# OmerKerner/noLZSS

Hardware: AMD Instinct MI355X
Metric: bases/sec factorized (1 GB sigma=4 DNA) + HBM GB/s fraction (higher is better)
Workload: dtype u32; 1 GPU; dna1g: one 2^30-base synthetic DNA sequence per GPU (sigma=4, 40% copied blocks, 1% substitutions), full factorization to (start,length,ref) records in HBM; bases_per_gpu=1073741824, parallelism=1 independent sequence shard(s), all-gather of counts

## Files before the change

include/nolzss_hip.h:

```cpp
#ifndef NOLZSS_HIP_H
#define NOLZSS_HIP_H

#include <stddef.h>
#include <stdint.h>

#ifdef __cplusplus
extern "C" {
#endif

typedef struct nolzss_factor {
    uint64_t start;
    uint64_t length;
    uint64_t ref;
} nolzss_factor;

#define NOLZSS_RC_MASK (1ULL << 63)

enum {
    NOLZSS_OK = 0,
    NOLZSS_ERR_INVALID_ARGUMENT = 1,
    NOLZSS_ERR_RUNTIME = 2,
    NOLZSS_ERR_NOMEM = 3,
    NOLZSS_ERR_DEVICE = 4,
    NOLZSS_ERR_IO = 5,
// ... 257 lines not shown
    uint64_t z, n_literals;
    uint64_t total_length;
    const uint64_t *target_lengths;
    int32_t device;
    uint64_t device_bytes;
} nolzss_rlz_archive_summary;
int nolzss_rlz_archive_open_records(const uint8_t *block, size_t block_len, const nolzss_factor *records, size_t z,
                                    const uint8_t *literals, size_t n_literals, const uint64_t *target_lengths,
                                    size_t k, int device, nolzss_rlz_archive **h);
int nolzss_rlz_archive_info(const nolzss_rlz_archive *h, nolzss_rlz_archive_summary *info);
int nolzss_rlz_archive_extract(const nolzss_rlz_archive *h, const nolzss_rlz_range *ranges, size_t q, uint8_t **bytes,
                               uint64_t **offsets, uint64_t *total);
int nolzss_rlz_archive_extract_device(const nolzss_rlz_archive *h, const nolzss_rlz_range *ranges, size_t q,
                                      void *d_out, size_t d_out_capacity, void *stream, uint64_t *total);
int nolzss_rlz_archive_close(nolzss_rlz_archive *h);

typedef struct nolzss_rlz_index nolzss_rlz_index;
typedef struct nolzss_rlz_index_summary {
    uint64_t num_references, block_length, index_length;
    int32_t with_rc, device;
    uint32_t prefix_syms;
    uint64_t device_bytes;
} nolzss_rlz_index_summary;
int nolzss_rlz_index_open(const char *const *refs, const size_t *ref_lens, size_t m, int with_rc,
                          uint32_t prefix_syms, int device, nolzss_rlz_index **h);
int nolzss_rlz_index_open_fasta(const char *reference_fasta_path, int with_rc, int sanitize_mode,
                                uint32_t prefix_syms, int device, nolzss_rlz_index **h);
int nolzss_rlz_index_info(const nolzss_rlz_index *h, nolzss_rlz_index_summary *info);
int nolzss_rlz_index_factorize(const nolzss_rlz_index *h, const char *const *targets, const size_t *target_lens,
                               size_t k, int want_factors, nolzss_rlz_result *out);
int nolzss_rlz_index_codes(const nolzss_rlz_index *h, const char *const *targets, const size_t *target_lens,
                           size_t k, uint32_t *code);
typedef struct nolzss_rlz_hit {
    uint64_t position;
    uint32_t record;
    uint32_t is_rc;
} nolzss_rlz_hit;
int nolzss_rlz_index_count(const nolzss_rlz_index *h, const char *const *patterns, const size_t *pattern_lens, size_t q,
                           uint64_t *counts);
int nolzss_rlz_index_locate(const nolzss_rlz_index *h, const char *const *patterns, const size_t *pattern_lens, size_t q,
                            uint64_t max_hits, uint64_t *counts, uint64_t *hit_offsets, nolzss_rlz_hit **hits,
                            size_t *num_hits);
int nolzss_debug_rlz_locate_shifts(uint64_t block_length, uint64_t q, int *shifts, int *npasses);
int nolzss_rlz_index_close(nolzss_rlz_index *h);

typedef struct nolzss_rlz_archive_append_info {
    uint64_t targets_added, records_added, literals_added, bases_added;
    uint64_t num_targets, z, total_length;
    uint64_t capacity_records;
    uint64_t device_bytes;
    int32_t reallocated;
} nolzss_rlz_archive_append_info;
int nolzss_rlz_archive_open_index(const nolzss_rlz_index *ix, nolzss_rlz_archive **h);
int nolzss_rlz_archive_append_index(nolzss_rlz_archive *h, const nolzss_rlz_index *ix, const char *const *targets,
                                    const size_t *target_lens, size_t k, nolzss_rlz_archive_append_info *info);
int nolzss_rlz_archive_export(const nolzss_rlz_archive *h, uint8_t **block, size_t *block_len, nolzss_factor **records,
                              size_t *z, uint8_t **literals, size_t *n_literals);

int nolzss_profile_enable(int device, int on);
int nolzss_profile_reset(int device);
int nolzss_profile_report(int device, char *buf, size_t cap);

int nolzss_debug_arrays(const uint8_t *text, size_t n, int device, uint32_t *sa, uint32_t *isa,
                        uint32_t *lcp, uint32_t *lstar);
int nolzss_debug_position_factors(const uint8_t *text, size_t n, int device, nolzss_factor *out);
int nolzss_debug_rc_arrays(const uint8_t *S, size_t S_len, int device, int want_plain, uint32_t *sa, uint32_t *isa,
                           uint32_t *lcp, uint32_t *code, uint32_t *plain, nolzss_factor *records,
                           uint32_t *counters);
int nolzss_debug_sort_pairs(uint64_t *keys, uint32_t *vals, size_t n, int device);
int nolzss_debug_scan(uint32_t *data, size_t n, int mode, int device);
enum { NOLZSS_PYR_NEAREST_LEFT = 0, NOLZSS_PYR_NEAREST_RIGHT = 1, NOLZSS_PYR_RANGE = 2 };
int nolzss_debug_pyramid(const uint32_t *base, size_t len, int is_max, int mode, const uint32_t *level1,
                         size_t first_entry, uint32_t flag_min, int poison, const uint32_t *queries, size_t nq,
                         int device, int *nlev, uint32_t *level_lens, uint32_t *levels, size_t levels_cap,
                         uint32_t *flag, uint32_t *results);
enum {
    NOLZSS_NEAR_UP_LESS = 0, NOLZSS_NEAR_UP_GREATER = 1, NOLZSS_NEAR_DOWN_LESS = 2, NOLZSS_NEAR_DOWN_GREATER = 3,
    NOLZSS_NEAR_FAR_UP_LESS = 4, NOLZSS_NEAR_FAR_UP_GREATER = 5, NOLZSS_NEAR_FAR_DOWN_LESS = 6,
    NOLZSS_NEAR_FAR_DOWN_GREATER = 7, NOLZSS_NEAR_LCP_INTERVAL = 8, NOLZSS_NEAR_LPNF_LEFTMOST = 9,
    NOLZSS_NEAR_LPNF_SEARCH = 10
};
int nolzss_debug_nearest(const uint32_t *sa, const uint32_t *lcp, size_t n, int poison, const uint32_t *queries,
                         size_t nq, int device, uint32_t *results);
int nolzss_debug_arena(int device, size_t *capacity, size_t *peak);
int nolzss_debug_parse_fasta(const char *path, int sanitize_mode, char **ids, size_t *ids_bytes,
                             char **sequences, size_t *sequences_bytes, size_t *count);
int nolzss_debug_parse_nucleotide_fasta(const char *path, char **ids, size_t *ids_bytes, char **sequences,
                                        size_t *sequences_bytes, size_t *count);
int nolzss_debug_lpt_plan(const size_t *lens, size_t m, size_t bins, size_t *owners);
int nolzss_debug_batch_plan(const size_t *lens, size_t m, size_t n_dev, int with_rc, int32_t *chunk_of, int32_t *device_of,
                            size_t *n_chunks);
int nolzss_debug_trim_arenas(int device, size_t *released_bytes);
void nolzss_debug_batch_counters(uint64_t *merged_records, uint64_t *single_records);

#ifdef __cplusplus
}
#endif
#endif
```

nolzss_amd/_lib.py:

```python
import ctypes as C
import os
from pathlib import Path

_PKG = Path(__file__).resolve().parent
LIB_PATH = Path(os.environ["NOLZSS_LIB"]).resolve() if os.environ.get("NOLZSS_LIB") else _PKG / "libnolzss_hip.so"

OK, ERR_INVALID_ARGUMENT, ERR_RUNTIME, ERR_NOMEM, ERR_DEVICE, ERR_IO, ERR_UNSUPPORTED = range(7)


class FastaResult(C.Structure):
    _fields_ = [("factors", C.c_void_p), ("num_factors", C.c_size_t),
                ("sentinel_factor_indices", C.c_void_p), ("num_sentinels", C.c_size_t),
                ("sequence_ids", C.c_void_p), ("sequence_ids_bytes", C.c_size_t),
                ("num_sequences", C.c_size_t)]


class FastaPerSequenceResult(C.Structure):
    _fields_ = [("factors", C.POINTER(C.c_void_p)), ("counts", C.POINTER(C.c_size_t)),
                ("sequence_ids", C.c_void_p), ("sequence_ids_bytes", C.c_size_t), ("num_sequences", C.c_size_t)]


class NucleotideFasta(C.Structure):
    _fields_ = [("sequence_ids", C.c_void_p), ("sequence_ids_bytes", C.c_size_t), ("num_sequences", C.c_size_t),
                ("lengths", C.POINTER(C.c_size_t)), ("counts", C.POINTER(C.c_size_t)),
# ... 159 lines not shown
    lib.nolzss_factorize_batch_dna_w_rc.argtypes = lib.nolzss_factorize_batch.argtypes
    lib.nolzss_factorize_batch_device.argtypes = [C.POINTER(C.c_void_p), C.POINTER(C.c_size_t), sz, C.c_int, C.c_int,
                                                  C.POINTER(C.c_size_t)]
    lib.nolzss_count_factors_batch_both.argtypes = [C.POINTER(C.c_void_p), C.POINTER(C.c_size_t), sz, C.POINTER(C.c_int),
                                                    sz, szp, szp]
    lib.nolzss_free_batch.argtypes = [C.POINTER(C.c_void_p), C.POINTER(C.c_size_t), sz]
    lib.nolzss_free_batch.restype = None
    lib.nolzss_read_nucleotide_fasta.argtypes = [C.c_char_p, C.POINTER(C.c_int), sz, C.c_int, sz, sz,
                                                 C.POINTER(NucleotideFasta)]
    lib.nolzss_free_nucleotide_fasta.argtypes = [C.POINTER(NucleotideFasta)]
    lib.nolzss_free_nucleotide_fasta.restype = None
    lib.nolzss_debug_parse_nucleotide_fasta.argtypes = [C.c_char_p, C.POINTER(C.c_void_p), szp, C.POINTER(C.c_void_p),
                                                        szp, szp]
    lib.nolzss_debug_lpt_plan.argtypes = [szp, sz, sz, szp]
    lib.nolzss_debug_batch_plan.argtypes = [szp, sz, sz, C.c_int, C.POINTER(C.c_int32), C.POINTER(C.c_int32), szp]
    lib.nolzss_free_length_hist.argtypes = [C.POINTER(LengthHist)]
    lib.nolzss_free_length_hist.restype = None
    lib.nolzss_factor_length_histogram.argtypes = [vp, sz, C.c_int, C.c_int, C.c_uint64, C.c_int, C.POINTER(LengthHist)]
    lib.nolzss_factor_length_histogram_with_lengths.argtypes = [vp, sz, C.c_int, C.c_int, C.POINTER(LengthHist)]
    lib.nolzss_fasta_factor_length_histogram.argtypes = [C.c_char_p, C.c_int, C.c_int, C.c_int, C.c_uint64, C.c_int,
                                                         C.POINTER(LengthHist)]
    lib.nolzss_fasta_factor_length_histogram_with_lengths.argtypes = [C.c_char_p, C.c_int, C.c_int, C.c_int,
                                                                      C.POINTER(LengthHist)]
    lib.nolzss_fasta_shuffled_text.argtypes = [C.c_char_p, C.c_int, C.c_int, C.c_uint64, C.c_int, vpp, szp]
    lib.nolzss_factor_lengths.argtypes = [vp, sz, C.c_int, C.c_int, vpp, szp]
    lib.nolzss_shuffle_dna.argtypes = [vp, sz, C.c_uint64, C.c_int, vpp]
    rqp, fmp = C.POINTER(FactorMapRequest), C.POINTER(FactorMaps)
    lib.nolzss_free_factor_maps.argtypes = [fmp]
    lib.nolzss_free_factor_maps.restype = None
    lib.nolzss_factor_maps_text.argtypes = [vp, sz, C.c_int, C.c_int, rqp, fmp]
    lib.nolzss_factor_maps_fasta.argtypes = [C.c_char_p, C.c_int, C.c_int, C.c_int, rqp, fmp]
    lib.nolzss_factor_maps_records.argtypes = [vp, sz, vp, sz, C.c_int, rqp, fmp]
    lib.nolzss_dotplot_open_text.argtypes = [vp, sz, C.c_int, C.c_int, vpp]
    lib.nolzss_dotplot_open_fasta.argtypes = [C.c_char_p, C.c_int, C.c_int, C.c_int, vpp]
    lib.nolzss_dotplot_open_records.argtypes = [vp, sz, vp, sz, C.c_int, vpp]
    lib.nolzss_dotplot_info.argtypes = [vp, C.POINTER(DotPlotSummary)]
    lib.nolzss_dotplot_render.argtypes = [vp, C.POINTER(DotPlotView), C.POINTER(DotPlotRaster)]
    lib.nolzss_free_dotplot_raster.argtypes = [C.POINTER(DotPlotRaster)]
    lib.nolzss_free_dotplot_raster.restype = None
    lib.nolzss_dotplot_close.argtypes = [vp]
    lib.nolzss_debug_position_edges.argtypes = [C.c_uint64, C.c_uint32, C.c_uint64, vpp, szp]
    seqs = [C.POINTER(C.c_char_p), szp, sz, C.POINTER(C.c_char_p), szp, sz]
    lib.nolzss_rlz_prepare.argtypes = seqs + [C.c_int, vpp, szp, vpp, szp, szp, szp]
    lib.nolzss_rlz_factorize.argtypes = seqs + [C.c_int, C.c_int, C.c_int, C.POINTER(RlzResult)]
    lib.nolzss_rlz_factorize_fasta.argtypes = [C.c_char_p, C.c_char_p, C.c_int, C.c_int, C.c_int, C.c_int,
                                               C.POINTER(RlzResult)]
    lib.nolzss_free_rlz_result.argtypes = [C.POINTER(RlzResult)]
    lib.nolzss_free_rlz_result.restype = None
    lib.nolzss_debug_rlz_codes.argtypes = seqs + [C.c_int, C.c_int, vp]
    u64p, dip = C.POINTER(C.c_uint64), C.POINTER(DecodeInfo)
    lib.nolzss_literal_symbols.argtypes = [vp, sz, vp, sz, vpp, szp]
    lib.nolzss_decode.argtypes = [vp, sz, vp, sz, vp, sz, C.c_int, vpp, szp, dip]
    lib.nolzss_roundtrip.argtypes = [vp, sz, C.c_int, C.c_int, szp, u64p, u64p, dip]
    lib.nolzss_roundtrip_device.argtypes = [vp, sz, C.c_int, C.c_int, vp, szp, u64p, u64p, dip]
    lib.nolzss_debug_count_mismatches.argtypes = [vp, vp, sz, C.c_int, u64p, u64p]
    lib.nolzss_rlz_archive_open_records.argtypes = [vp, sz, vp, sz, vp, sz, vp, sz, C.c_int, vpp]
    lib.nolzss_rlz_archive_info.argtypes = [vp, C.POINTER(RlzArchiveSummary)]
    lib.nolzss_rlz_archive_extract.argtypes = [vp, vp, sz, vpp, vpp, u64p]
    lib.nolzss_rlz_archive_extract_device.argtypes = [vp, vp, sz, vp, sz, vp, u64p]
    lib.nolzss_rlz_archive_close.argtypes = [vp]
    lib.nolzss_rlz_index_open.argtypes = seqs[:3] + [C.c_int, C.c_uint32, C.c_int, vpp]
    lib.nolzss_rlz_index_open_fasta.argtypes = [C.c_char_p, C.c_int, C.c_int, C.c_uint32, C.c_int, vpp]
    lib.nolzss_rlz_index_info.argtypes = [vp, C.POINTER(RlzIndexSummary)]
    lib.nolzss_rlz_index_factorize.argtypes = [vp] + seqs[3:] + [C.c_int, C.POINTER(RlzResult)]
    lib.nolzss_rlz_index_codes.argtypes = [vp] + seqs[3:] + [vp]
    lib.nolzss_rlz_index_close.argtypes = [vp]
    lib.nolzss_rlz_index_count.argtypes = [vp] + seqs[3:] + [vp]
    lib.nolzss_rlz_index_locate.argtypes = [vp] + seqs[3:] + [C.c_uint64, vp, vp, vpp, szp]
    lib.nolzss_debug_rlz_locate_shifts.argtypes = [C.c_uint64, C.c_uint64, C.POINTER(C.c_int), C.POINTER(C.c_int)]
    lib.nolzss_rlz_archive_open_index.argtypes = [vp, vpp]
    lib.nolzss_rlz_archive_append_index.argtypes = [vp, vp] + seqs[3:] + [C.POINTER(RlzArchiveAppendInfo)]
    lib.nolzss_rlz_archive_export.argtypes = [vp, vpp, szp, vpp, szp, vpp, szp]
    lib.nolzss_profile_enable.argtypes = [C.c_int, C.c_int]
    lib.nolzss_profile_reset.argtypes = [C.c_int]
    lib.nolzss_profile_report.argtypes = [C.c_int, C.c_char_p, sz]
    lib.nolzss_debug_arrays.argtypes = [vp, sz, C.c_int, vp, vp, vp, vp]
    lib.nolzss_debug_position_factors.argtypes = [vp, sz, C.c_int, vp]
    lib.nolzss_debug_rc_arrays.argtypes = [vp, sz, C.c_int, C.c_int, vp, vp, vp, vp, vp, vp, vp]
    lib.nolzss_debug_sort_pairs.argtypes = [vp, vp, sz, C.c_int]
    lib.nolzss_debug_scan.argtypes = [vp, sz, C.c_int, C.c_int]
    lib.nolzss_debug_pyramid.argtypes = [vp, sz, C.c_int, C.c_int, vp, sz, C.c_uint32, C.c_int, vp, sz, C.c_int,
                                         C.POINTER(C.c_int), vp, vp, sz, vp, vp]
    lib.nolzss_debug_nearest.argtypes = [vp, vp, sz, C.c_int, vp, sz, C.c_int, vp]
    lib.nolzss_debug_arena.argtypes = [C.c_int, szp, szp]
    lib.nolzss_debug_trim_arenas.argtypes = [C.c_int, szp]
    lib.nolzss_debug_parse_fasta.argtypes = [C.c_char_p, C.c_int, C.POINTER(C.c_void_p), szp, C.POINTER(C.c_void_p),
                                             szp, szp]
    lib.nolzss_debug_batch_counters.argtypes = [C.POINTER(C.c_uint64), C.POINTER(C.c_uint64)]
    lib.nolzss_debug_batch_counters.restype = None
    return lib


lib = _load()

EXPORTED_SYMBOLS = [
    "nolzss_last_error", "nolzss_version", "nolzss_free", "nolzss_device_count",
    "nolzss_factorize", "nolzss_count_factors", "nolzss_factorize_file", "nolzss_count_factors_file",
    "nolzss_factorize_device", "nolzss_prepare_multiple_dna_w_rc",
    "nolzss_factorize_multiple_dna_w_rc", "nolzss_count_factors_multiple_dna_w_rc",
    "nolzss_factorize_dna_w_rc", "nolzss_count_factors_dna_w_rc", "nolzss_factorize_batch",
    "nolzss_factorize_w_reference", "nolzss_factorize_dna_w_reference_seq",
    "nolzss_write_factors_binary_file", "nolzss_write_factors_binary_file_dna_w_rc",
    "nolzss_factorize_w_reference_file", "nolzss_factorize_dna_w_reference_seq_file",
    "nolzss_write_factor_file", "nolzss_prepare_multiple_dna_no_rc", "nolzss_factorize_fasta_multiple_dna",
    "nolzss_free_fasta_result", "nolzss_write_factors_binary_file_fasta_multiple_dna",
    "nolzss_factorize_fasta_per_sequence", "nolzss_free_fasta_per_sequence_result",
    "nolzss_factorize_dna_rc_w_ref_fasta_files", "nolzss_write_factors_dna_w_reference_fasta_files_to_binary",
    "nolzss_free_batch", "nolzss_profile_enable", "nolzss_profile_reset", "nolzss_profile_report",
    "nolzss_debug_arrays", "nolzss_debug_sort_pairs", "nolzss_debug_scan", "nolzss_debug_arena",
    "nolzss_debug_batch_counters", "nolzss_factorize_batch_dna_w_rc",
    "nolzss_debug_trim_arenas", "nolzss_debug_parse_fasta",
    "nolzss_read_nucleotide_fasta", "nolzss_free_nucleotide_fasta", "nolzss_debug_parse_nucleotide_fasta", "nolzss_debug_lpt_plan", "nolzss_debug_batch_plan", "nolzss_factorize_batch_device",
    "nolzss_factorize_dna_w_rc_device", "nolzss_count_factors_batch_both",
    "nolzss_free_length_hist", "nolzss_factor_length_histogram", "nolzss_factor_length_histogram_with_lengths",
    "nolzss_fasta_factor_length_histogram", "nolzss_fasta_factor_length_histogram_with_lengths",
    "nolzss_fasta_shuffled_text", "nolzss_factor_lengths", "nolzss_shuffle_dna",
    "nolzss_free_factor_maps", "nolzss_factor_maps_text", "nolzss_factor_maps_fasta", "nolzss_factor_maps_records",
    "nolzss_debug_position_edges",
    "nolzss_dotplot_open_text", "nolzss_dotplot_open_fasta", "nolzss_dotplot_open_records", "nolzss_dotplot_info",
    "nolzss_dotplot_render", "nolzss_free_dotplot_raster", "nolzss_dotplot_close",
    "nolzss_debug_position_factors", "nolzss_debug_rc_arrays",
    "nolzss_rlz_prepare", "nolzss_rlz_factorize", "nolzss_rlz_factorize_fasta", "nolzss_free_rlz_result",
    "nolzss_debug_rlz_codes",
    "nolzss_literal_symbols", "nolzss_decode", "nolzss_roundtrip", "nolzss_roundtrip_device",
    "nolzss_debug_count_mismatches",
    "nolzss_rlz_archive_open_records", "nolzss_rlz_archive_info", "nolzss_rlz_archive_extract",
    "nolzss_rlz_archive_extract_device", "nolzss_rlz_archive_close",
    "nolzss_rlz_index_open", "nolzss_rlz_index_open_fasta", "nolzss_rlz_index_info", "nolzss_rlz_index_factorize",
    "nolzss_rlz_index_codes", "nolzss_rlz_index_close", "nolzss_rlz_index_count", "nolzss_rlz_index_locate",
    "nolzss_debug_rlz_locate_shifts",
    "nolzss_rlz_archive_open_index", "nolzss_rlz_archive_append_index", "nolzss_rlz_archive_export",
    "nolzss_debug_pyramid", "nolzss_debug_nearest",
]


def check(rc):
    if rc == OK:
        return
    msg = lib.nolzss_last_error().decode("utf-8", "replace")
    if rc == ERR_INVALID_ARGUMENT:
        raise ValueError(msg)
    if rc == ERR_NOMEM:
        raise MemoryError(msg)
    raise RuntimeError(msg)
```

nolzss_amd/_noLZSS.py:

```python
import ctypes as C
import operator
import os

import numpy as np

from . import _lib
from ._lib import lib, check

__version__ = lib.nolzss_version().decode()

RC_MASK = 1 << 63
FACTOR_DTYPE = np.dtype([("start", "<u8"), ("length", "<u8"), ("ref", "<u8")])
HIT_DTYPE = np.dtype([("position", "<u8"), ("record", "<u4"), ("is_rc", "<u4")])

_default_device = int(os.environ.get("NOLZSS_DEVICE", os.environ.get("LOCAL_RANK", "0")) or 0)


def set_device(device: int) -> None:
    global _default_device
    _default_device = int(device)


def get_device() -> int:
    return _default_device
# ... 1361 lines not shown
    return list(zip(a, b))


def debug_lpt_plan(lengths, bins: int):
    m = len(lengths)
    lens = (C.c_size_t * max(m, 1))(*lengths)
    owners = (C.c_size_t * max(m, 1))()
    check(lib.nolzss_debug_lpt_plan(lens, m, bins, owners))
    return [owners[j] for j in range(m)]


def debug_batch_plan(lengths, n_dev: int, with_rc: bool = False):
    m = len(lengths)
    lens = (C.c_size_t * max(m, 1))(*lengths)
    chunk_of = (C.c_int32 * max(m, 1))()
    device_of = (C.c_int32 * max(m, 1))()
    n_chunks = C.c_size_t()
    check(lib.nolzss_debug_batch_plan(lens, m, n_dev, 1 if with_rc else 0, chunk_of, device_of, C.byref(n_chunks)))
    return [chunk_of[j] for j in range(m)], [device_of[j] for j in range(m)], n_chunks.value


def debug_trim_arenas() -> int:
    r = C.c_size_t()
    check(lib.nolzss_debug_trim_arenas(_default_device, C.byref(r)))
    return r.value


def debug_batch_counters():
    a, b = C.c_uint64(), C.c_uint64()
    lib.nolzss_debug_batch_counters(C.byref(a), C.byref(b))
    return a.value, b.value


def debug_scan(data, mode: int):
    data = np.ascontiguousarray(data, dtype=np.uint32).copy()
    check(lib.nolzss_debug_scan(data.ctypes.data, data.size, mode, _default_device))
    return data


PYR_NEAREST_LEFT, PYR_NEAREST_RIGHT, PYR_RANGE = range(3)
(NEAR_UP_LESS, NEAR_UP_GREATER, NEAR_DOWN_LESS, NEAR_DOWN_GREATER, NEAR_FAR_UP_LESS, NEAR_FAR_UP_GREATER,
 NEAR_FAR_DOWN_LESS, NEAR_FAR_DOWN_GREATER, NEAR_LCP_INTERVAL, NEAR_LPNF_LEFTMOST, NEAR_LPNF_SEARCH) = range(11)


def debug_pyramid(base, is_max: bool, queries=None, mode: int = 0, level1=None, first_entry: int = 0,
                  flag_min: int = 0, poison: int = 0, want_levels: bool = True):
    base = np.ascontiguousarray(base, dtype=np.uint32)
    q = np.ascontiguousarray(queries if queries is not None else np.zeros((0, 3)), dtype=np.uint32).reshape(-1, 3)
    l1 = np.ascontiguousarray(level1, dtype=np.uint32) if level1 is not None else None
    if l1 is not None and l1.size < first_entry:
        raise ValueError("level1 holds fewer than first_entry entries")
    lens, length = [], base.size
    while True:
        lens.append(length)
        if length <= 1 or len(lens) == 9:
            break
        length = (length + 15) >> 4
    levels = np.zeros(max(sum(lens), 1), dtype=np.uint32)
    got_lens = np.zeros(9, dtype=np.uint32)
    nlev, flag = C.c_int(), C.c_uint32()
    results = np.zeros(max(len(q), 1), dtype=np.uint32)
    check(lib.nolzss_debug_pyramid(base.ctypes.data, base.size, 1 if is_max else 0, mode,
                                   l1.ctypes.data if l1 is not None else None, first_entry, flag_min, poison,
                                   q.ctypes.data, len(q), _default_device, C.byref(nlev), got_lens.ctypes.data,
                                   levels.ctypes.data if want_levels else None, levels.size, C.byref(flag),
                                   results.ctypes.data))
    got_lens = [int(v) for v in got_lens[:nlev.value]]
    ends = np.cumsum(got_lens)
    return {"nlev": nlev.value, "lens": got_lens,
            "levels": [levels[e - n:e] for e, n in zip(ends, got_lens)] if want_levels else None,
            "flag": flag.value, "results": results[:len(q)]}


def debug_nearest(sa, lcp, queries, poison: int = 0):
    sa = np.ascontiguousarray(sa, dtype=np.uint32)
    lcp = np.ascontiguousarray(lcp, dtype=np.uint32)
    if lcp.size != sa.size + 1:
        raise ValueError("lcp must hold one entry more than sa")
    q = np.ascontiguousarray(queries, dtype=np.uint32).reshape(-1, 5)
    results = np.zeros((max(len(q), 1), 2), dtype=np.uint32)
    check(lib.nolzss_debug_nearest(sa.ctypes.data, lcp.ctypes.data, sa.size, poison, q.ctypes.data, len(q),
                                   _default_device, results.ctypes.data))
    return results[:len(q)]
```

nolzss_amd/csrc/debug_pyramid.hip:

```cpp
#include "api_internal.hpp"
#include "nearest.hpp"

using namespace nolzss;
using namespace nolzss::api;

namespace {

constexpr int kQueryThreads = 256;
constexpr size_t kSpare = 16;

template <bool kMax>
__global__ __launch_bounds__(kQueryThreads) void debug_pyramid_query_kernel(Pyramid P, const uint32_t *__restrict__ q,
                                                                            size_t nq, uint32_t *__restrict__ out) {
    const size_t stride = (size_t)gridDim.x * blockDim.x;
    for (size_t k = (size_t)blockIdx.x * blockDim.x + threadIdx.x; k < nq; k += stride) {
        const uint32_t op = q[3 * k], a = q[3 * k + 1], b = q[3 * k + 2];
        uint32_t res;
        if (op == NOLZSS_PYR_NEAREST_LEFT)
            res = (uint32_t)pyr_nearest_left<kMax>(P, a, b);
        else if (op == NOLZSS_PYR_NEAREST_RIGHT)
            res = pyr_nearest_right<kMax>(P, a, b);
        else
            res = pyr_range<kMax>(P, a, b);
        out[k] = res;
    }
}

__global__ __launch_bounds__(kQueryThreads) void debug_nearest_query_kernel(const uint32_t *__restrict__ sa,
                                                                            const uint32_t *__restrict__ lcp, uint32_t n,
                                                                            Pyramid Pmin, Pyramid Pmax, Pyramid Plcp,
                                                                            const uint32_t *__restrict__ q, size_t nq,
                                                                            uint32_t *__restrict__ out) {
    const size_t stride = (size_t)gridDim.x * blockDim.x;
    for (size_t k = (size_t)blockIdx.x * blockDim.x + threadIdx.x; k < nq; k += stride) {
        const uint32_t op = q[5 * k], r = q[5 * k + 1], a = q[5 * k + 2], b = q[5 * k + 3], c = q[5 * k + 4];
        uint32_t o0 = 0, o1 = 0;
        switch (op) {
        case NOLZSS_NEAR_UP_LESS: nearest_up<false>(sa, lcp, Pmin, Plcp, r, a, b, o0, o1); break;
        case NOLZSS_NEAR_UP_GREATER: nearest_up<true>(sa, lcp, Pmax, Plcp, r, a, b, o0, o1); break;
        case NOLZSS_NEAR_DOWN_LESS: nearest_down<false>(sa, lcp, n, Pmin, Plcp, r, a, b, o0, o1); break;
        case NOLZSS_NEAR_DOWN_GREATER: nearest_down<true>(sa, lcp, n, Pmax, Plcp, r, a, b, o0, o1); break;
        case NOLZSS_NEAR_FAR_UP_LESS: far_up<false>(sa, Pmin, Plcp, r, a, b, o0, o1); break;
        case NOLZSS_NEAR_FAR_UP_GREATER: far_up<true>(sa, Pmax, Plcp, r, a, b, o0, o1); break;
        case NOLZSS_NEAR_FAR_DOWN_LESS: far_down<false>(sa, n, Pmin, Plcp, r, a, b, o0, o1); break;
        case NOLZSS_NEAR_FAR_DOWN_GREATER: far_down<true>(sa, n, Pmax, Plcp, r, a, b, o0, o1); break;
        case NOLZSS_NEAR_LCP_INTERVAL: lcp_interval(Plcp, r, a, o0, o1); break;
        case NOLZSS_NEAR_LPNF_LEFTMOST: o0 = lpnf_leftmost(Pmin, Plcp, r, a); break;
        default: o0 = lpnf_search(Pmin, Plcp, r, a, b, c); break;
        }
        out[2 * k] = o0;
        out[2 * k + 1] = o1;
    }
}

size_t padded_bytes(size_t entries) { return (entries * sizeof(uint32_t) + 255) & ~size_t(255); }

int level_lengths(uint32_t len, uint32_t *lens) {
    int nlev = 1;
    lens[0] = len;
    while (lens[nlev - 1] > 1 && nlev < kPyrMaxLevels) {
        lens[nlev] = (lens[nlev - 1] + kPyrFan - 1) >> kPyrShift;
        ++nlev;
    }
    return nlev;
}

size_t upper_level_bytes(uint32_t len) {
    uint32_t lens[kPyrMaxLevels];
    const int nlev = level_lengths(len, lens);
    size_t bytes = 0;
    for (int l = 1; l < nlev; ++l) bytes += padded_bytes(lens[l]);
    return bytes;
}

uint32_t *upload_poisoned(Context &ctx, const uint32_t *h, size_t len, int poison) {
    uint32_t *d = ctx.arena.alloc<uint32_t>(len + kSpare);
    HIP_CHECK(hipMemsetAsync(d, poison, padded_bytes(len + kSpare), ctx.stream));
    HIP_CHECK(hipMemcpyAsync(d, h, len * sizeof(uint32_t), hipMemcpyHostToDevice, ctx.stream));
    return d;
}

void poison_ahead(Context &ctx, size_t bytes, int poison) {
    if (bytes == 0) return;
    const size_t mark = ctx.arena.mark();
    uint8_t *scratch = ctx.arena.alloc<uint8_t>(bytes);
    HIP_CHECK(hipMemsetAsync(scratch, poison, bytes, ctx.stream));
    ctx.arena.rewind(mark);
}

unsigned query_grid(size_t nq) {
    const size_t g = div_up(nq, (size_t)kQueryThreads);
    return (unsigned)(g > 1024 ? 1024 : g);
}

void check_poison(int poison) {
    if (poison != 0x00 && poison != 0xFF) throw std::invalid_argument("poison must be 0x00 or 0xFF");
}

}

extern "C" {

int nolzss_debug_pyramid(const uint32_t *base, size_t len, int is_max, int mode, const uint32_t *level1,
                         size_t first_entry, uint32_t flag_min, int poison, const uint32_t *queries, size_t nq,
                         int device, int *nlev, uint32_t *level_lens, uint32_t *levels, size_t levels_cap,
                         uint32_t *flag, uint32_t *results) {
    return guarded([&] {
        if (!base || !nlev || !level_lens) throw std::invalid_argument("null argument");
        if (len == 0) throw std::invalid_argument("the base array is empty");
        if (len >= (size_t(1) << 32)) throw std::invalid_argument("the base array has 2^32 entries or more");
        if (mode != 0 && mode != 1) throw std::invalid_argument("build mode must be 0 or 1");
        check_poison(poison);
        if (nq && (!queries || !results)) throw std::invalid_argument("null query or result array");
        if (flag_min != 0 && (is_max || mode != 0 || !flag || len < 2))
            throw std::invalid_argument("flag_min is for a min pyramid with a level 1, built in mode 0, with a flag word to return");
        uint32_t lens[kPyrMaxLevels];
        const int levels_n = level_lengths((uint32_t)len, lens);
        size_t total = 0;
        for (int l = 0; l < levels_n; ++l) total += lens[l];
        if (levels && levels_cap < total) throw std::invalid_argument("the level buffer is too small");
        if (mode == 1) {
            if (len < 2) throw std::invalid_argument("mode 1 needs a level 1: at least 2 entries");
            if (first_entry > lens[1]) throw std::invalid_argument("first_entry lies beyond level 1");
            if (first_entry && !level1) throw std::invalid_argument("null level-1 array");
        }
        for (size_t k = 0; k < nq; ++k) {
            const uint32_t op = queries[3 * k], a = queries[3 * k + 1], b = queries[3 * k + 2];
            if (op == NOLZSS_PYR_NEAREST_LEFT) {
                if (a >= len) throw std::invalid_argument("nearest_left: r is not below len");
            } else if (op == NOLZSS_PYR_RANGE) {
                if (a > b || b >= len) throw std::invalid_argument("range: needs a <= b < len");
            } else if (op != NOLZSS_PYR_NEAREST_RIGHT) {
                throw std::invalid_argument("unknown pyramid query");
            }
// ... 7 lines not shown
        uint32_t *d_flag = ctx.arena.alloc<uint32_t>(1);
        HIP_CHECK(hipMemsetAsync(d_flag, 0, sizeof(uint32_t), s));
        uint32_t *d_q = nq ? ctx.arena.alloc<uint32_t>(3 * nq) : nullptr;
        uint32_t *d_res = nq ? ctx.arena.alloc<uint32_t>(nq) : nullptr;
        const uint32_t *d_base = upload_poisoned(ctx, base, len, poison);
        poison_ahead(ctx, upper_level_bytes((uint32_t)len), poison);
        Pyramid P;
        if (mode == 0) {
            P = build_pyramid(d_base, (uint32_t)len, is_max != 0, ctx.arena, s, flag_min, flag_min ? d_flag : nullptr);
        } else {
            P = alloc_pyramid(d_base, (uint32_t)len, ctx.arena);
            if (first_entry)
                HIP_CHECK(hipMemcpyAsync(const_cast<uint32_t *>(P.lvl[1]), level1, first_entry * sizeof(uint32_t),
                                         hipMemcpyHostToDevice, s));
            fill_pyramid_tail(P, (uint32_t)first_entry, is_max != 0, s);
            fill_pyramid(P, 2, is_max != 0, s);
        }
        if (P.nlev != levels_n) throw std::logic_error("debug_pyramid: level count differs from alloc_pyramid's");
        if (nq) {
            HIP_CHECK(hipMemcpyAsync(d_q, queries, 3 * nq * sizeof(uint32_t), hipMemcpyHostToDevice, s));
            if (is_max)
                debug_pyramid_query_kernel<true><<<query_grid(nq), kQueryThreads, 0, s>>>(P, d_q, nq, d_res);
            else
                debug_pyramid_query_kernel<false><<<query_grid(nq), kQueryThreads, 0, s>>>(P, d_q, nq, d_res);
            KERNEL_CHECK();
            HIP_CHECK(hipMemcpyAsync(results, d_res, nq * sizeof(uint32_t), hipMemcpyDeviceToHost, s));
        }
        *nlev = P.nlev;
        size_t at = 0;
        for (int l = 0; l < P.nlev; ++l) {
            level_lens[l] = P.len[l];
            if (levels) HIP_CHECK(hipMemcpyAsync(levels + at, P.lvl[l], P.len[l] * sizeof(uint32_t), hipMemcpyDeviceToHost, s));
            at += P.len[l];
        }
        if (flag) HIP_CHECK(hipMemcpyAsync(flag, d_flag, sizeof(uint32_t), hipMemcpyDeviceToHost, s));
        HIP_CHECK(hipStreamSynchronize(s));
        ctx.arena.rewind(mark);
    });
}

int nolzss_debug_nearest(const uint32_t *sa, const uint32_t *lcp, size_t n, int poison, const uint32_t *queries,
                         size_t nq, int device, uint32_t *results) {
    return guarded([&] {
        if (!sa || !lcp) throw std::invalid_argument("null argument");
        if (n == 0) throw std::invalid_argument("the arrays are empty");
        if (n + 1 >= (size_t(1) << 32)) throw std::invalid_argument("the LCP array has 2^32 entries or more");
        check_poison(poison);
        if (lcp[0] != 0 || lcp[n] != 0) throw std::invalid_argument("lcp[0] and lcp[n] must be 0");
        if (nq && (!queries || !results)) throw std::invalid_argument("null query or result array");
        for (size_t k = 0; k < nq; ++k) {
            const uint32_t op = queries[5 * k], r = queries[5 * k + 1], a = queries[5 * k + 2];
            if (op > NOLZSS_NEAR_LPNF_SEARCH) throw std::invalid_argument("unknown search");
            if (r >= n) throw std::invalid_argument("search: r is not below n");
            if ((op == NOLZSS_NEAR_LCP_INTERVAL || op == NOLZSS_NEAR_LPNF_LEFTMOST) && a < 1)
                throw std::invalid_argument("lcp_interval / lpnf_leftmost: d must be at least 1");
            if (op == NOLZSS_NEAR_LPNF_SEARCH && a >= n) throw std::invalid_argument("lpnf_search: i is not below n");
        }
        if (nq == 0) return;

        Session ses(device, nullptr);
        Context &ctx = ses.ctx();
        const size_t upper = 2 * upper_level_bytes((uint32_t)n) + upper_level_bytes((uint32_t)n + 1);
        ctx.arena.reserve(padded_bytes(n + kSpare) + padded_bytes(n + 1 + kSpare) + upper + nq * 32 + (size_t(64) << 20));
        const size_t mark = ctx.arena.mark();
        hipStream_t s = ctx.stream;
        uint32_t *d_q = ctx.arena.alloc<uint32_t>(5 * nq);
        uint32_t *d_res = ctx.arena.alloc<uint32_t>(2 * nq);
        const uint32_t *d_sa = upload_poisoned(ctx, sa, n, poison);
        const uint32_t *d_lcp = upload_poisoned(ctx, lcp, n + 1, poison);
        poison_ahead(ctx, upper, poison);
        const Pyramid Pmin = build_pyramid(d_sa, (uint32_t)n, false, ctx.arena, s);
        const Pyramid Pmax = build_pyramid(d_sa, (uint32_t)n, true, ctx.arena, s);
        const Pyramid Plcp = build_pyramid(d_lcp, (uint32_t)n + 1, false, ctx.arena, s);
        HIP_CHECK(hipMemcpyAsync(d_q, queries, 5 * nq * sizeof(uint32_t), hipMemcpyHostToDevice, s));
        debug_nearest_query_kernel<<<query_grid(nq), kQueryThreads, 0, s>>>(d_sa, d_lcp, (uint32_t)n, Pmin, Pmax, Plcp, d_q,
                                                                           nq, d_res);
        KERNEL_CHECK();
        HIP_CHECK(hipMemcpyAsync(results, d_res, 2 * nq * sizeof(uint32_t), hipMemcpyDeviceToHost, s));
        HIP_CHECK(hipStreamSynchronize(s));
        ctx.arena.rewind(mark);
    });
}

}
```

nolzss_amd/csrc/nearest_lds.hpp:

```cpp
#pragma once
#include "nearest.hpp"

#include <type_traits>

namespace nolzss {

constexpr int kLdsThreads = 256;
constexpr int kLdsWaves = kLdsThreads / 64;
constexpr int kLdsTile = 1024;
constexpr int kLdsPerWave = kLdsTile / kLdsWaves;
constexpr int kLdsReach = 256;
constexpr int kLdsSpan = kLdsTile + 2 * kLdsReach;
constexpr int kLdsStep0 = 4;
constexpr uint32_t kFarLen = 0xffffffffu;
__device__ __forceinline__ uint32_t far_mark(uint32_t m, uint32_t far_bit) {
    return far_bit ? (far_bit | (m & ~far_bit)) : kFarLen;
}
__device__ __forceinline__ bool far_is(uint32_t v, uint32_t far_bit) {
    return far_bit ? (v & far_bit) != 0 : v == kFarLen;
}
__device__ __forceinline__ uint32_t far_bound(uint32_t v, uint32_t far_bit) {
    return far_bit ? (v & ~far_bit) : 0xffffffffu;
}
__device__ __forceinline__ bool far_resolve(uint32_t &up, uint32_t &down, uint32_t far_bit, uint32_t floor_len) {
// ... 38 lines not shown
    }
    if (pending) atomicOr(flag, 1u);
}

constexpr uint16_t kNoMatch = 0xffffu;
__device__ __forceinline__ uint32_t match_pos(const uint32_t *s_sa, uint16_t at) { return at == kNoMatch ? kNoPos : s_sa[at]; }
template <int kSteps, bool kGreater, bool kUp>
__device__ __forceinline__ int lds_scan_round(const uint32_t *s_sa, const uint32_t *s_lcp, int li, int s0, uint32_t x,
                                              uint32_t &m, uint32_t &at) {
    uint32_t c[kSteps], v[kSteps];
#pragma unroll
    for (int k = 0; k < kSteps; ++k) {
        const int q = kUp ? li - (s0 + k + 1) : li + (s0 + k + 1);
        c[k] = s_lcp[q + (kUp ? 1 : 0)];
        v[k] = s_sa[q];
    }
    bool alive = true;
    uint32_t kk = 0;
#pragma unroll
    for (int k = 0; k < kSteps; ++k) {
        const uint32_t mk = c[k] < m ? c[k] : m;
        const bool qual = kGreater ? v[k] > x : v[k] < x;
        const bool stop = alive && qual;
        m = alive ? mk : m;
        kk = stop ? (uint32_t)k : kk;
        alive = alive != stop;
    }
    at = (uint32_t)(kUp ? li - (s0 + (int)kk + 1) : li + (s0 + (int)kk + 1));
    return m == 0 ? 0 : (alive ? 2 : 1);
}

constexpr int kBlk = 16;
constexpr int kNumBlk = kLdsSpan / kBlk;
static_assert(kLdsSpan % kBlk == 0 && kLdsReach % kBlk == 0 && kLdsTile % kBlk == 0, "aligned blocks");
constexpr int kStepA = 12;
static_assert(kLdsStep0 + kStepA + 1 >= kBlk, "round B would look at the rank itself and at ranks on its other side");

constexpr int kBlkTableLen = kNumBlk + 2;
struct BlockTables {
    uint32_t *mn, *mx;
    uint32_t *lup, *ldn;
};
template <bool kMax> __device__ __forceinline__ BlockTables block_tables(uint32_t *mem) {
    if (kMax) return BlockTables{mem + 1, mem + kBlkTableLen + 1, mem + 2 * kBlkTableLen + 1, mem + 3 * kBlkTableLen + 1};
    return BlockTables{mem + 1, nullptr, mem + kBlkTableLen + 1, mem + 2 * kBlkTableLen + 1};
}

template <bool kMax>
__device__ __forceinline__ void build_block_tables(const uint32_t *s_sa, const uint32_t *s_lcp, const BlockTables &T) {
    const int B = (int)threadIdx.x;
    if (B < kNumBlk) {
        const uint4 *p = reinterpret_cast<const uint4 *>(s_sa + kBlk * B);
        const uint4 *c = reinterpret_cast<const uint4 *>(s_lcp + kBlk * B);
        uint32_t mn = 0xffffffffu, mx = 0u, lo = 0xffffffffu;
        uint32_t first = 0;
#pragma unroll
        for (int q = 0; q < 4; ++q) {
            const uint4 a = p[q], l = c[q];
            const uint32_t av[4] = {a.x, a.y, a.z, a.w}, lv[4] = {l.x, l.y, l.z, l.w};
#pragma unroll
            for (int e = 0; e < 4; ++e) {
                mn = av[e] < mn ? av[e] : mn;
                mx = av[e] > mx ? av[e] : mx;
                if (q == 0 && e == 0)
                    first = lv[e];
                else
                    lo = lv[e] < lo ? lv[e] : lo;
            }
        }
        const uint32_t last = s_lcp[kBlk * B + kBlk];
        T.mn[B] = mn;
        if (kMax) T.mx[B] = mx;
        T.ldn[B] = lo < first ? lo : first;
        T.lup[B] = lo < last ? lo : last;
    } else if (B < kNumBlk + 2) {
        const int o = B == kNumBlk ? -1 : kNumBlk;
        T.mn[o] = 0xffffffffu;
        if (kMax) T.mx[o] = 0u;
        T.ldn[o] = 0xffffffffu;
        T.lup[o] = 0xffffffffu;
    }
}

constexpr uint32_t kListOverflow = 0xffffffffu;
template <bool kGreater, bool kUp, bool kHasPos, int kListCapB, typename ThrGt>
__device__ __forceinline__ void lds_search_tail(const uint32_t *s_sa, const uint32_t *s_lcp, const BlockTables &T, int w,
                                                uint32_t *res_len, uint16_t *res_pos, const uint16_t *list, uint32_t cnt,
                                                uint16_t *list_b, ThrGt thr_gt, uint32_t far_bit) {
    static_assert(kListCapB >= 64, "a step of round A appends up to 64 searches");
    const int lane = lane_id();
    const uint64_t lt = lanemask_lt();
    const uint32_t *tv = kGreater ? T.mx : T.mn;
    const uint32_t *tc = kUp ? T.lup : T.ldn;
    auto rounds_bc = [&](uint32_t cnt_b) {
        __builtin_amdgcn_fence(__ATOMIC_RELEASE, "wavefront");
        __builtin_amdgcn_wave_barrier();
        for (uint32_t c0 = 0; c0 < cnt_b; c0 += 64) {
            const bool have = c0 + lane < cnt_b;
            const int tl = have ? (int)list_b[c0 + lane] : 0;
            const int t = w * kLdsPerWave + tl;
            const int li = t + kLdsReach;
            const uint32_t i = s_sa[li];
            const uint32_t x = kGreater ? thr_gt(i) : i;
            const int b0 = kUp ? (li - (kLdsStep0 + kStepA + 1)) >> 4 : (li + (kLdsStep0 + kStepA + 1)) >> 4;
            uint32_t c[kBlk], v[kBlk];
#pragma unroll
            for (int j = 0; j < kBlk; ++j) {
                const int B = kUp ? b0 - j : b0 + j;
                c[j] = tc[B];
                v[j] = tv[B];
            }
            uint32_t run = have ? res_len[t] : 0xffffffffu;
            int jstar = -1;
            bool alive = true;
#pragma unroll
            for (int j = 0; j < kBlk; ++j) {
                const uint32_t rk = c[j] < run ? c[j] : run;
                const bool qual = kGreater ? v[j] > x : v[j] < x;
                const bool stop = alive && qual;
                jstar = stop ? j : jstar;
                alive = alive != stop;
                run = alive ? rk : run;
            }
            const bool inside = have && jstar >= 0;
            const int Bs = kUp ? b0 - jstar : b0 + jstar;
            const int anchor = inside ? (kUp ? kBlk * Bs + kBlk : kBlk * Bs - 1) : li;
            uint32_t m = run, at = 0;
            const int st = lds_scan_round<kBlk, kGreater, kUp>(s_sa, s_lcp, anchor, 0, x, m, at);
            if (have) {
                res_len[t] = inside ? m : far_mark(run, far_bit);
                if (kHasPos) res_pos[t] = (inside && st == 1) ? (uint16_t)at : kNoMatch;
            }
        }
        __builtin_amdgcn_fence(__ATOMIC_RELEASE, "wavefront");
        __builtin_amdgcn_wave_barrier();
    };
    uint32_t cnt_b = 0;
    for (uint32_t c0 = 0; c0 < cnt; c0 += 64) {
        if (kListCapB < kLdsPerWave && cnt_b + 64 > (uint32_t)kListCapB) {
            rounds_bc(cnt_b);
            cnt_b = 0;
        }
        const bool have = c0 + lane < cnt;
        const int tl = have ? (int)list[c0 + lane] : 0;
        const int t = w * kLdsPerWave + tl;
        const int li = t + kLdsReach;
        bool pending = false;
        if (have) {
            const uint32_t i = s_sa[li];
            uint32_t m = res_len[t], at = 0;
            const int st = lds_scan_round<kStepA, kGreater, kUp>(s_sa, s_lcp, li, kLdsStep0, kGreater ? thr_gt(i) : i, m, at);
            pending = st == 2;
            res_len[t] = m;
            if (kHasPos) res_pos[t] = (st == 1) ? (uint16_t)at : kNoMatch;
        }
        const uint64_t bal = __ballot(pending);
        if (pending) list_b[cnt_b + (uint32_t)__popcll(bal & lt)] = (uint16_t)tl;
        cnt_b += (uint32_t)__popcll(bal);
    }
    rounds_bc(cnt_b);
}

template <int NS, int NP, bool kCompact = false, int kListCap = kLdsPerWave, int kListCapB = kListCap, typename Active, typename ThrGt>
__device__ __forceinline__ void lds_search_wave_blocks(const uint32_t *s_sa, const uint32_t *s_lcp,
                                                       const BlockTables &T, uint32_t n, uint32_t base,
                                                       uint32_t *res_len, uint16_t *res_pos, uint16_t *list0,
                                                       uint16_t *list1, Active active, ThrGt thr_gt,
                                                       uint32_t far_bit, unsigned long long *phase_clock = nullptr) {
    static_assert(NS == 2 || NS == 4, "searches: smaller up / down, then greater up / down");
    const int lane = lane_id();
    const int w = threadIdx.x >> 6;
    const uint64_t lt = lanemask_lt();
    uint32_t cnt[NS];
#pragma unroll
    for (int k = 0; k < NS; ++k) cnt[k] = 0;

    uint32_t rows = kLdsPerWave / 64, n_act = kLdsPerWave;
    if (kCompact) {
        n_act = 0;
#pragma unroll
        for (int row = 0; row < kLdsPerWave / 64; ++row) {
            const int tl = row * 64 + lane;
            const int t = w * kLdsPerWave + tl;
            const bool valid = (uint64_t)base + t < n && active(s_sa[t + kLdsReach]);
            const uint64_t bal = __ballot(valid);
            if (valid) list1[n_act + (uint32_t)__popcll(bal & lt)] = (uint16_t)tl;
            n_act += (uint32_t)__popcll(bal);
        }
        __builtin_amdgcn_fence(__ATOMIC_RELEASE, "wavefront");
        __builtin_amdgcn_wave_barrier();
        rows = (n_act + 63) / 64;
    }
#pragma unroll 1
    for (uint32_t row = 0; row < rows; ++row) {
        const bool have = !kCompact || row * 64 + lane < n_act;
        const int tl = kCompact ? (have ? (int)list1[row * 64 + lane] : 0) : (int)(row * 64 + lane);
        const int t = w * kLdsPerWave + tl;
        const uint64_t rr = (uint64_t)base + t;
        const int li = t + kLdsReach;
        const uint32_t i = s_sa[li];
        const bool valid = kCompact ? have : (rr < n && active(i));
        auto search = [&](auto kk) {
            constexpr int k = decltype(kk)::value;
            constexpr bool greater = k >= 2, up = (k & 1) == 0;
            uint32_t m = 0xffffffffu, at = 0;
            int st = 0;
            if (valid) st = lds_scan_round<kLdsStep0, greater, up>(s_sa, s_lcp, li, 0, greater ? thr_gt(i) : i, m, at);
            if (have) {
                res_len[k * kLdsTile + t] = (st == 0) ? 0u : m;
                if (k < NP) res_pos[k * kLdsTile + t] = (st == 1) ? (uint16_t)at : kNoMatch;
            }
            const bool pending = st == 2;
            const uint64_t bal = __ballot(pending);
            const uint32_t slot = cnt[k] + (uint32_t)__popcll(bal & lt);
// ... 37 lines not shown
```

Baseline: 13.93 billion bases/s.

## Split LDS block-table search rounds across lane groups with DPP reductions

Rounds B and C of the LDS nearest-smaller/greater search now assign each pending query to a group of 2 or 4 lanes instead of one lane. Each lane scans a slice of the block tables and of the final in-block scan, and the group combines results through ballot-based first-stop detection and DPP min/max reductions. The aim is to cut the serial per-lane scan length and register pressure for the tail searches, in exchange for extra cross-lane operations and fewer queries per wave iteration. A debug entry point and Python binding are added to test the kernel.

```diff
diff --git a/include/nolzss_hip.h b/include/nolzss_hip.h
--- a/include/nolzss_hip.h
+++ b/include/nolzss_hip.h
@@ -363,6 +363,10 @@
 };
 int nolzss_debug_nearest(const uint32_t *sa, const uint32_t *lcp, size_t n, int poison, const uint32_t *queries,
                          size_t nq, int device, uint32_t *results);
+enum { NOLZSS_LDS_PLAIN = 0, NOLZSS_LDS_RC = 1 };
+#define NOLZSS_LDS_OVERFLOW 0xffffffffu
+int nolzss_debug_lds_search(const uint32_t *sa, const uint32_t *lcp, size_t n, int form, uint32_t strand, int poison,
+                            int device, uint32_t *len, uint32_t *pos);
 int nolzss_debug_arena(int device, size_t *capacity, size_t *peak);
 int nolzss_debug_parse_fasta(const char *path, int sanitize_mode, char **ids, size_t *ids_bytes,
                              char **sequences, size_t *sequences_bytes, size_t *count);
diff --git a/nolzss_amd/_lib.py b/nolzss_amd/_lib.py
--- a/nolzss_amd/_lib.py
+++ b/nolzss_amd/_lib.py
@@ -265,6 +265,7 @@
     lib.nolzss_debug_pyramid.argtypes = [vp, sz, C.c_int, C.c_int, vp, sz, C.c_uint32, C.c_int, vp, sz, C.c_int,
                                          C.POINTER(C.c_int), vp, vp, sz, vp, vp]
     lib.nolzss_debug_nearest.argtypes = [vp, vp, sz, C.c_int, vp, sz, C.c_int, vp]
+    lib.nolzss_debug_lds_search.argtypes = [vp, vp, sz, C.c_int, C.c_uint32, C.c_int, C.c_int, vp, vp]
     lib.nolzss_debug_arena.argtypes = [C.c_int, szp, szp]
     lib.nolzss_debug_trim_arenas.argtypes = [C.c_int, szp]
     lib.nolzss_debug_parse_fasta.argtypes = [C.c_char_p, C.c_int, C.POINTER(C.c_void_p), szp, C.POINTER(C.c_void_p),
@@ -313,7 +314,7 @@
     "nolzss_rlz_index_codes", "nolzss_rlz_index_close", "nolzss_rlz_index_count", "nolzss_rlz_index_locate",
     "nolzss_debug_rlz_locate_shifts",
     "nolzss_rlz_archive_open_index", "nolzss_rlz_archive_append_index", "nolzss_rlz_archive_export",
-    "nolzss_debug_pyramid", "nolzss_debug_nearest",
+    "nolzss_debug_pyramid", "nolzss_debug_nearest", "nolzss_debug_lds_search",
 ]
 
 
diff --git a/nolzss_amd/_noLZSS.py b/nolzss_amd/_noLZSS.py
--- a/nolzss_amd/_noLZSS.py
+++ b/nolzss_amd/_noLZSS.py
@@ -1467,3 +1467,20 @@
     check(lib.nolzss_debug_nearest(sa.ctypes.data, lcp.ctypes.data, sa.size, poison, q.ctypes.data, len(q),
                                    _default_device, results.ctypes.data))
     return results[:len(q)]
+
+
+LDS_PLAIN, LDS_RC = 0, 1
+LDS_OVERFLOW = 0xffffffff
+
+
+def debug_lds_search(sa, lcp, form: int = LDS_PLAIN, strand: int = 0, poison: int = 0):
+    sa = np.ascontiguousarray(sa, dtype=np.uint32)
+    lcp = np.ascontiguousarray(lcp, dtype=np.uint32)
+    if lcp.size != sa.size + 1:
+        raise ValueError("lcp must hold one entry more than sa")
+    searches = 4 if form == LDS_RC else 2
+    length = np.zeros((searches, max(sa.size, 1)), dtype=np.uint32)
+    pos = np.zeros((2, max(sa.size, 1)), dtype=np.uint32)
+    check(lib.nolzss_debug_lds_search(sa.ctypes.data, lcp.ctypes.data, sa.size, form, strand, poison, _default_device,
+                                      length.ctypes.data, pos.ctypes.data))
+    return length, pos
diff --git a/nolzss_amd/csrc/debug_pyramid.hip b/nolzss_amd/csrc/debug_pyramid.hip
--- a/nolzss_amd/csrc/debug_pyramid.hip
+++ b/nolzss_amd/csrc/debug_pyramid.hip
@@ -1,5 +1,6 @@
 #include "api_internal.hpp"
 #include "nearest.hpp"
+#include "nearest_lds.hpp"
 
 using namespace nolzss;
 using namespace nolzss::api;
@@ -50,6 +51,48 @@
         }
         out[2 * k] = o0;
         out[2 * k + 1] = o1;
+    }
+}
+
+template <bool kRc>
+__global__ __launch_bounds__(kLdsThreads) void debug_lds_search_kernel(const uint32_t *__restrict__ sa,
+                                                                       const uint32_t *__restrict__ lcp, uint32_t n,
+                                                                       uint32_t N, uint32_t *__restrict__ out_len,
+                                                                       uint32_t *__restrict__ out_pos) {
+    constexpr int NS = kRc ? 4 : 2, NP = 2;
+    constexpr int kListCap = kRc ? 128 : kLdsPerWave;
+    constexpr int kListCapB = 64;
+    __shared__ __align__(16) uint32_t s_sa[kLdsSpan];
+    __shared__ __align__(16) uint32_t s_lcp[kLdsSpan + 4];
+    __shared__ uint32_t s_len[NS * kLdsTile];
+    __shared__ uint16_t s_pos[NP * kLdsTile];
+    __shared__ uint16_t s_list0[kLdsWaves][NS * kListCap];
+    __shared__ uint16_t s_list1[kLdsWaves][NS * kListCapB];
+    __shared__ uint32_t s_blk[(kRc ? 4 : 3) * kBlkTableLen];
+    const uint32_t base = blockIdx.x * (uint32_t)kLdsTile;
+    stage_tile(sa, lcp, n, base, s_sa, s_lcp);
+    __syncthreads();
+    const BlockTables T = block_tables<kRc>(s_blk);
+    build_block_tables<kRc>(s_sa, s_lcp, T);
+    __syncthreads();
+    const int w = threadIdx.x >> 6;
+    const uint32_t far_bit = n <= 0x80000000u ? 0x80000000u : 0u;
+    if constexpr (kRc)
+        lds_search_wave_blocks<NS, NP, true, kListCap, kListCapB>(s_sa, s_lcp, T, n, base, s_len, s_pos, s_list0[w], s_list1[w],
+                                       [N](uint32_t i) { return i < N; }, [N](uint32_t i) { return 2u * N - i; }, far_bit);
+    else
+        lds_search_wave_blocks<NS, NP, false, kListCap, kListCapB>(s_sa, s_lcp, T, n, base, s_len, s_pos, s_list0[w], s_list1[w],
+                                       [](uint32_t) { return true; }, [](uint32_t) { return 0u; }, far_bit);
+    for (int row = 0; row < kLdsPerWave / 64; ++row) {
+        const int t = w * kLdsPerWave + row * 64 + lane_id();
+        const uint64_t rr = (uint64_t)base + t;
+        if (rr >= n) continue;
+        const bool searched = !kRc || s_sa[t + kLdsReach] < N;
+#pragma unroll
+        for (int k = 0; k < NS; ++k) {
+            out_len[(size_t)k * n + rr] = searched ? s_len[k * kLdsTile + t] : 0u;
+            if (k < NP) out_pos[(size_t)k * n + rr] = searched ? match_pos(s_sa, s_pos[k * kLdsTile + t]) : kNoPos;
+        }
     }
 }
 
@@ -223,4 +266,38 @@
     });
 }
 
-}
+int nolzss_debug_lds_search(const uint32_t *sa, const uint32_t *lcp, size_t n, int form, uint32_t strand, int poison,
+                            int device, uint32_t *len, uint32_t *pos) {
+    return guarded([&] {
+        if (!sa || !lcp || !len || !pos) throw std::invalid_argument("null argument");
+        if (n == 0) throw std::invalid_argument("the arrays are empty");
+        if (n > (size_t(1) << 31) - 2 * kLdsTile) throw std::invalid_argument("more than 2^31 - 2048 ranks");
+        if (form != NOLZSS_LDS_PLAIN && form != NOLZSS_LDS_RC) throw std::invalid_argument("unknown form of the LDS searches");
+        check_poison(poison);
+        if (lcp[0] != 0 || lcp[n] != 0) throw std::invalid_argument("lcp[0] and lcp[n] must be 0");
+        const size_t searches = form == NOLZSS_LDS_RC ? 4 : 2;
+
+        Session ses(device, nullptr);
+        Context &ctx = ses.ctx();
+        ctx.arena.reserve(padded_bytes(n + kSpare) + padded_bytes(n + 1 + kSpare) + (searches + 2) * padded_bytes(n) +
+                          (size_t(64) << 20));
+        const size_t mark = ctx.arena.mark();
+        hipStream_t s = ctx.stream;
+        uint32_t *d_len = ctx.arena.alloc<uint32_t>(searches * n);
+        uint32_t *d_pos = ctx.arena.alloc<uint32_t>(2 * n);
+        const uint32_t *d_sa = upload_poisoned(ctx, sa, n, poison);
+        const uint32_t *d_lcp = upload_poisoned(ctx, lcp, n + 1, poison);
+        const unsigned tiles = (unsigned)div_up(n, (size_t)kLdsTile);
+        if (form == NOLZSS_LDS_RC)
+            debug_lds_search_kernel<true><<<tiles, kLdsThreads, 0, s>>>(d_sa, d_lcp, (uint32_t)n, strand, d_len, d_pos);
+        else
+            debug_lds_search_kernel<false><<<tiles, kLdsThreads, 0, s>>>(d_sa, d_lcp, (uint32_t)n, strand, d_len, d_pos);
+        KERNEL_CHECK();
+        HIP_CHECK(hipMemcpyAsync(len, d_len, searches * n * sizeof(uint32_t), hipMemcpyDeviceToHost, s));
+        HIP_CHECK(hipMemcpyAsync(pos, d_pos, 2 * n * sizeof(uint32_t), hipMemcpyDeviceToHost, s));
+        HIP_CHECK(hipStreamSynchronize(s));
+        ctx.arena.rewind(mark);
+    });
+}
+
+}
diff --git a/nolzss_amd/csrc/nearest_lds.hpp b/nolzss_amd/csrc/nearest_lds.hpp
--- a/nolzss_amd/csrc/nearest_lds.hpp
+++ b/nolzss_amd/csrc/nearest_lds.hpp
@@ -144,6 +144,46 @@
     }
 }
 
+#ifndef NOLZSS_LANES_BC
+#define NOLZSS_LANES_BC 4
+#endif
+constexpr int kLanesBC = NOLZSS_LANES_BC;
+static_assert(kLanesBC == 2 || kLanesBC == 4, "a group of lanes lies inside a DPP quad");
+constexpr int kPerLaneBC = kBlk / kLanesBC;
+
+template <typename Op> __device__ __forceinline__ uint32_t group_reduce_bc(uint32_t v, Op op) {
+    v = op(v, (uint32_t)__builtin_amdgcn_update_dpp(0, (int)v, 0xB1, 0xf, 0xf, true));
+    if (kLanesBC == 4) v = op(v, (uint32_t)__builtin_amdgcn_update_dpp(0, (int)v, 0x4E, 0xf, 0xf, true));
+    return v;
+}
+struct OpMaxU32 {
+    __device__ __forceinline__ uint32_t operator()(uint32_t a, uint32_t b) const { return a > b ? a : b; }
+};
+__device__ __forceinline__ bool stop_in_front_bc(bool stop, int lane, uint32_t ahead) {
+    const uint64_t bal = __ballot(stop);
+    const uint32_t half = lane < 32 ? (uint32_t)bal : (uint32_t)(bal >> 32);
+    return (half & ahead) != 0;
+}
+
+template <int kSteps, bool kGreater, bool kThrough>
+__device__ __forceinline__ bool lds_scan_share(const uint32_t (&c)[kSteps], const uint32_t (&v)[kSteps], uint32_t x, uint32_t &m,
+                                               uint32_t &kk) {
+    bool alive = true;
+    m = 0xffffffffu;
+    kk = 0;
+#pragma unroll
+    for (int k = 0; k < kSteps; ++k) {
+        const uint32_t mk = c[k] < m ? c[k] : m;
+        const bool qual = kGreater ? v[k] > x : v[k] < x;
+        const bool stop = alive && qual;
+        if (kThrough) m = alive ? mk : m;
+        kk = stop ? (uint32_t)k : kk;
+        alive = alive != stop;
+        if (!kThrough) m = alive ? mk : m;
+    }
+    return !alive;
+}
+
 constexpr uint32_t kListOverflow = 0xffffffffu;
 template <bool kGreater, bool kUp, bool kHasPos, int kListCapB, typename ThrGt>
 __device__ __forceinline__ void lds_search_tail(const uint32_t *s_sa, const uint32_t *s_lcp, const BlockTables &T, int w,
@@ -154,44 +194,54 @@
     const uint64_t lt = lanemask_lt();
     const uint32_t *tv = kGreater ? T.mx : T.mn;
     const uint32_t *tc = kUp ? T.lup : T.ldn;
+    const int q = lane & (kLanesBC - 1);
+    const uint32_t ahead = ((1u << q) - 1u) << (lane & 31 & ~(kLanesBC - 1));
     auto rounds_bc = [&](uint32_t cnt_b) {
         __builtin_amdgcn_fence(__ATOMIC_RELEASE, "wavefront");
         __builtin_amdgcn_wave_barrier();
-        for (uint32_t c0 = 0; c0 < cnt_b; c0 += 64) {
-            const bool have = c0 + lane < cnt_b;
-            const int tl = have ? (int)list_b[c0 + lane] : 0;
+        for (uint32_t c0 = 0; c0 < cnt_b; c0 += 64 / kLanesBC) {
+            const bool have = c0 + (uint32_t)(lane / kLanesBC) < cnt_b;
+            const int tl = have ? (int)list_b[c0 + (uint32_t)(lane / kLanesBC)] : 0;
             const int t = w * kLdsPerWave + tl;
             const int li = t + kLdsReach;
             const uint32_t i = s_sa[li];
             const uint32_t x = kGreater ? thr_gt(i) : i;
             const int b0 = kUp ? (li - (kLdsStep0 + kStepA + 1)) >> 4 : (li + (kLdsStep0 + kStepA + 1)) >> 4;
-            uint32_t c[kBlk], v[kBlk];
-#pragma unroll
-            for (int j = 0; j < kBlk; ++j) {
-                const int B = kUp ? b0 - j : b0 + j;
+            const int Bq = kUp ? b0 - q * kPerLaneBC : b0 + q * kPerLaneBC;
+            uint32_t c[kPerLaneBC], v[kPerLaneBC];
+#pragma unroll
+            for (int j = 0; j < kPerLaneBC; ++j) {
+                const int B = kUp ? Bq - j : Bq + j;
                 c[j] = tc[B];
                 v[j] = tv[B];
             }
-            uint32_t run = have ? res_len[t] : 0xffffffffu;
-            int jstar = -1;
-            bool alive = true;
-#pragma unroll
-            for (int j = 0; j < kBlk; ++j) {
-                const uint32_t rk = c[j] < run ? c[j] : run;
-                const bool qual = kGreater ? v[j] > x : v[j] < x;
-                const bool stop = alive && qual;
-                jstar = stop ? j : jstar;
-                alive = alive != stop;
-                run = alive ? rk : run;
-            }
-            const bool inside = have && jstar >= 0;
-            const int Bs = kUp ? b0 - jstar : b0 + jstar;
-            const int anchor = inside ? (kUp ? kBlk * Bs + kBlk : kBlk * Bs - 1) : li;
-            uint32_t m = run, at = 0;
-            const int st = lds_scan_round<kBlk, kGreater, kUp>(s_sa, s_lcp, anchor, 0, x, m, at);
-            if (have) {
+            uint32_t part, jq;
+            const bool stop_b = lds_scan_share<kPerLaneBC, kGreater, false>(c, v, x, part, jq);
+            const bool late_b = stop_in_front_bc(stop_b, lane, ahead);
+            const uint32_t carry = have ? res_len[t] : 0xffffffffu;
+            const uint32_t rest = group_reduce_bc(late_b ? 0xffffffffu : part, OpMinU32());
+            const uint32_t run = carry < rest ? carry : rest;
+            const int Bmine = kUp ? Bq - (int)jq : Bq + (int)jq;
+            const uint32_t Bs1 = group_reduce_bc((stop_b && !late_b) ? (uint32_t)(Bmine + 1) : 0u, OpMaxU32());
+            const bool inside = have && Bs1 != 0;
+            const int Bs = (int)Bs1 - 1;
+            const int first = kUp ? kBlk * Bs + kBlk : kBlk * Bs - 1;
+            const int anchor = inside ? (kUp ? first - q * kPerLaneBC : first + q * kPerLaneBC) : li;
+#pragma unroll
+            for (int k = 0; k < kPerLaneBC; ++k) {
+                const int p = kUp ? anchor - (k + 1) : anchor + (k + 1);
+                c[k] = s_lcp[p + (kUp ? 1 : 0)];
+                v[k] = s_sa[p];
+            }
+            uint32_t mine, kq;
+            const bool stop_c = lds_scan_share<kPerLaneBC, kGreater, true>(c, v, x, mine, kq);
+            const bool late_c = stop_in_front_bc(stop_c, lane, ahead);
+            const uint32_t upto = group_reduce_bc(late_c ? 0xffffffffu : mine, OpMinU32());
+            const uint32_t m = run < upto ? run : upto;
+            if (inside ? (stop_c && !late_c) : (have && q == 0)) {
+                const uint32_t at = (uint32_t)(kUp ? anchor - ((int)kq + 1) : anchor + ((int)kq + 1));
                 res_len[t] = inside ? m : far_mark(run, far_bit);
-                if (kHasPos) res_pos[t] = (inside && st == 1) ? (uint16_t)at : kNoMatch;
+                if (kHasPos) res_pos[t] = (inside && m != 0) ? (uint16_t)at : kNoMatch;
             }
         }
         __builtin_amdgcn_fence(__ATOMIC_RELEASE, "wavefront");
```

Measured after the change: 14.13 billion bases/s, median of 6. +1.5%, better.
